# google-research/frame-interpolation

Measured on NVIDIA H100. Metric: interpolated_frames_per_sec_1080p, higher is better.
Workload: dtype f16x2-split (activations/weights as fp16 hi+lo planes; fp32 accumulate)

## Files before the change

frame_interpolation_b200/csrc/film_conv3x3_tc.cu:

```cuda
#include <cuda.h>
#include <cuda_runtime.h>
#include <stdint.h>

#include <type_traits>

#include "film_conv.h"
#include "film_tc_ptx.cuh"

namespace film {
namespace {
using namespace tc;

constexpr int kConsumers = 256;
constexpr int kThreads = kConsumers + 128;
__host__ __device__ constexpr int a_plane_bytes(int kc, int th, int tw) { return (th + 2) * tw * kc * 2; }
__host__ __device__ constexpr int a_stage_bytes(int kc, int th, int tw) { return 2 * a_plane_bytes(kc, th, tw); }
constexpr int kHaloW = 10;
__host__ __device__ constexpr int halo_box_bytes(int kc, int th) { return (th + 2) * kHaloW * kc * 2; }
__host__ __device__ constexpr int halo_plane_bytes(int kc, int th) { return (halo_box_bytes(kc, th) + 1023) & ~1023; }
__host__ __device__ constexpr int a_stage_bytes_h(int kc, int th, int tw, int halo, int planes = 2) {
  return planes * (halo ? halo_plane_bytes(kc, th) : a_plane_bytes(kc, th, tw));
}
constexpr int kMaxRing = 8;
constexpr int kSmemLimit = 227 * 1024;
constexpr int kBarBytes = 8 * (4 * kMaxRing + 4);
constexpr int kFixedBytes = kBarBytes + 16 + 512 * 4  + 64  + 1024  + 64;
constexpr int kHeadW3 = 64 * 32 * 4, kHeadMisc = 512;
constexpr int kHeadBytes = kHeadW3 + kHeadMisc;
constexpr int kPxnStageWg = 64 * 64 * 2;
constexpr int kPxnStageBytes = 2 * kPxnStageWg;
inline int epi_scratch_bytes(int epi_mode, int pxn) { return epi_mode == 3 ? kHeadBytes : pxn ? kPxnStageBytes : 0; }

__host__ __device__ inline int w_tap_bytes(int bn, int kc, int planes = 2) { return bn * kc * 2 * planes; }

template <int BN, int KC, bool kPartial, bool kHalo, bool kOne, bool kRes, bool kPxN = false>
__global__ void __launch_bounds__(kThreads, 1) k_conv3x3_tc(const ConvProblem* __restrict__ prob) {
  static_assert(!kPxN || (BN == 64 && KC == 64), "pixels on N: Cout = 64 (one M = 64 weight tile), 64-channel chunks");
  extern __shared__ uint8_t smem_raw[];
  constexpr bool one = kOne;
  const int planes = one ? 1 : 2;
  constexpr int kWPlane = BN * KC * 2;
  const int kWTap = kWPlane * planes;
  const int kTileH = prob->tile_h, kTileW = prob->tile_w;
  constexpr int kHaloTileH = kPxN ? 32 : 16;
  constexpr int kHaloBox = halo_box_bytes(KC, kHaloTileH), kHaloPlane = halo_plane_bytes(KC, kHaloTileH);
  constexpr bool halo = kHalo;
  const int kAPlane = halo ? kHaloPlane : a_plane_bytes(KC, kTileH, kTileW);
  const int kAStage = planes * kAPlane;
  const int kRowStep = kTileW * KC * 2;
  constexpr bool kFused = BN <= 128 && !kPxN;
  constexpr int kAccRegs = kPxN ? 64 : (kFused ? 2 * BN : BN) / 2;
  constexpr int kWgPx = kPxN ? 128 : 64;

  const int NA = prob->v2_na, NW = prob->v2_nw;
  const bool resident = prob->v2_resident != 0;
  const int nsrc = prob->nsrc;
  const int tiles_x = prob->tiles_x, tiles_per_img = prob->tiles_y * prob->tiles_x;
  const int cout = prob->cout;
  const int n_nt = (cout + BN - 1) / BN;
  const int ntiles = prob->B * tiles_per_img * n_nt;
  constexpr int kStageTaps = kHalo ? 9 : 3;
  constexpr bool kPacked = kPartial && kPxN;
  const int part_lo = prob->v2_part_lo, part_hi = prob->v2_part_hi;
  int nab = 0;
  for (int s = 0; s < nsrc; ++s) nab += prob->src[s].nchunk * (kHalo ? 1 : 3);
  const int nkb = nab * kStageTaps - (kPacked ? (part_hi - part_lo) * (kStageTaps - kStageTaps / 3) : 0);

  const FastDiv div_nt(n_nt, ntiles), div_img(tiles_per_img, ntiles), div_tx(tiles_x, ntiles);
  const bool pair = prob->pair != 0;
  const int rank = pair ? (int)cluster_ctarank() : 0;
  const int nsp = prob->B * tiles_per_img;
  const int nwork = pair ? ((nsp + 1) / 2) * n_nt : ntiles;
  const int w_first = pair ? (int)blockIdx.x >> 1 : (int)blockIdx.x, w_step = pair ? (int)gridDim.x >> 1 : (int)gridDim.x;
  auto decode = [&](int work, int& sp, int& nti) {
    div_nt.divmod(work, sp, nti);
    if (pair) sp = 2 * sp + rank;
  };

  const uint32_t raw = smem_u32(smem_raw);
  const uint32_t base = (raw + 1023u) & ~1023u;
  uint8_t* gen_base = smem_raw + (base - raw);
  const uint32_t a_base = base;
  const uint32_t w_base = a_base + (uint32_t)NA * kAStage;
  const uint32_t w_bytes = resident ? (uint32_t)nkb * kWTap : (uint32_t)NW * kWTap;
  const uint32_t tail = w_base + w_bytes;
  const uint32_t tail_off = (uint32_t)NA * kAStage + w_bytes;
  float* bias_smem = reinterpret_cast<float*>(gen_base + tail_off + kBarBytes + 16);
  int* src_tab = reinterpret_cast<int*>(gen_base + tail_off + kBarBytes + 16 + 512 * 4);

// ... 67 lines not shown
        __syncwarp();
      }
      int kb = 0, ab = 0;
      for (int s = 0; s < nsrc; ++s) {
        const int nchunk = src_tab[2 * s], c_off = src_tab[2 * s + 1];
        const int bs = src_tab[2 * kMaxSrc + s] ? prob->B - 1 - b : b;
        const CUtensorMap* tm_hi = &prob->tm_a_hi[s];
        const CUtensorMap* tm_lo = &prob->tm_a_lo[s];
        for (int ch = 0; ch < nchunk; ++ch) {
          const int nst = halo ? 1 : 3;
          for (int dx = 0; dx < nst; ++dx, ++ab) {
            const int st = ra.stage;
            mbar_wait(tail + 8u * (kMaxRing + st), ra.phase ^ 1u);
            if (elect_one()) {
              const uint32_t sa = a_base + st * kAStage, bar = tail + 8u * st;
              mbar_expect_tx(bar, halo ? (uint32_t)(planes * kHaloBox) : (uint32_t)kAStage);
              tma_load_4d(sa, tm_hi, bar, c_off + ch * KC, x0 + dx - 1, y0 - 1, bs);
              if (!one) tma_load_4d(sa + kAPlane, tm_lo, bar, c_off + ch * KC, x0 + dx - 1, y0 - 1, bs);
            }
            __syncwarp();
            ra.advance(NA);
            if (!resident) {
              const bool packed = kPacked && ab >= part_lo && ab < part_hi;
              const int nblk = packed ? kStageTaps / 3 : kStageTaps;
              for (int t = 0; t < nblk; ++t, ++kb) {
                const int ws = rw.stage;
                mbar_wait(tail + 8u * (3 * kMaxRing + ws), rw.phase ^ 1u);
                if (elect_one()) {
                  const uint32_t sw = w_base + ws * kWTap, bar = tail + 8u * (2 * kMaxRing + ws);
                  mbar_expect_tx(bar, kWTap);
                  if (pair) {
                    const uint32_t hoff = (uint32_t)(rank * (kWPlane / 2));
                    tma_load_2d_mc(sw + hoff, &prob->tm_w_hi_half, bar, kb * KC, n0 + rank * (BN / 2), 3);
                    if (!one) tma_load_2d_mc(sw + kWPlane + hoff, &prob->tm_w_lo_half, bar, kb * KC, n0 + rank * (BN / 2), 3);
                  } else {
                    tma_load_2d(sw, tm_w_hi, bar, kb * KC, n0);
                    if (!one) tma_load_2d(sw + kWPlane, tm_w_lo, bar, kb * KC, n0);
                  }
                }
                __syncwarp();
                rw.advance(NW);
              }
            }
          }
        }
      }
    }
    leave();
    return;
  }

  regs_inc<232>();
  const int wg = warp >> 2;
  const int q = lane & 3;
  const int H = prob->H, W = prob->W, out_H = prob->out_H, out_W = prob->out_W, out_C = prob->out_C;
  const int out_c_off = prob->out_c_off, act = prob->act;
  sp_t* const out_hi = prob->out_hi;
  sp_t* const out_lo = prob->out_lo;
  sp_t* const pool_hi = prob->pool_hi;
  sp_t* const pool_lo = prob->pool_lo;
  const int pool_C = prob->pool_C;
  const bool do_pool = pool_hi != nullptr;
  const bool lo_skip = prob->out_lo_skip != 0;
  const bool rgb = prob->epi_mode == 2;
  const float* const head_w = prob->head_w4;
  float* const rgb_out = prob->head_v;
  const int crop_y = prob->crop_y, crop_x = prob->crop_x, crop_h = prob->crop_h, crop_w = prob->crop_w;
  const int64_t crop_pitch = prob->crop_pitch;
  const bool fhead = prob->epi_mode == 3;
  constexpr int kHid = BN <= 64 ? BN / 2 : 1;
  float* const w3s = reinterpret_cast<float*>(reinterpret_cast<uint8_t*>(src_tab) + 64);
  float* const hmisc = w3s + kHeadW3 / 4;
  if (fhead) {
    if constexpr (BN <= 64) {
      for (int i = threadIdx.x; i < BN * kHid; i += kConsumers) w3s[i] = prob->head_w3[i];
      for (int i = threadIdx.x; i < kHid; i += kConsumers) hmisc[i] = prob->head_b3[i];
      for (int i = threadIdx.x; i < 2 * kHid; i += kConsumers) hmisc[kHid + i] = prob->head_w4[i];
      if (threadIdx.x < 2) hmisc[3 * kHid + threadIdx.x] = prob->head_b4[threadIdx.x];
    }
    asm volatile("bar.sync 1, %0;" ::"r"(kConsumers) : "memory");
  }
  const float* const head_vup = prob->head_vup;
  float* const head_res = prob->head_res;
  float* const head_vout = prob->head_v;

  if (resident) mbar_wait(tail + 8u * (2 * kMaxRing), 0);
  const bool is_leader = (threadIdx.x & 127) == 0;
  const uint32_t w_empty_peer = pair ? map_to_cta(tail + 8u * (3 * kMaxRing), (uint32_t)(rank ^ 1)) : 0u;
  auto release_w = [&](int slot) {
    mbar_arrive(tail + 8u * (3 * kMaxRing + slot));
    if (pair) mbar_arrive_cluster(w_empty_peer + 8u * slot);
  };
  {
    constexpr int kWTapC = kWPlane * (kOne ? 1 : 2);
    constexpr uint32_t kPx = KC * 2;
    const uint32_t a_row0 = kHalo ? (uint32_t)(wg * (kWgPx / 8) * kHaloW) * kPx : (uint32_t)(wg * kWgPx) * kPx;
    const uint32_t sbo = kHalo ? kHaloW * kPx : 8 * kPx;
    RingPos ra, rw;
    float acc[kAccRegs];
    for (int tile = w_first; tile < nwork; tile += w_step) {
      int kb = 0;
      int rel_a = -1, rel_w = -1;
      auto retire = [&](int next_a, int next_w) {
        wgmma_commit();
        wgmma_wait<1>();
        if (is_leader) {
          if (rel_a >= 0) mbar_arrive(tail + 8u * (kMaxRing + rel_a));
          if (rel_w >= 0) release_w(rel_w);
        }
        rel_a = next_a;
        rel_w = next_w;
      };
      auto stage = [&](auto ksteps_c, auto tpb_c) {
        constexpr int kSteps = decltype(ksteps_c)::value, kTpb = decltype(tpb_c)::value;
        constexpr int kBlocks = kStageTaps / kTpb;
        const int st = ra.stage;
        mbar_wait(tail + 8u * st, ra.phase);
        const uint32_t sa = a_base + st * kAStage + a_row0;
        const uint32_t lo_off = (uint32_t)(kHalo ? kHaloPlane : kAPlane);
        if constexpr (kRes) {
          const uint64_t a0 = make_desc_sbo<KC>(sa, sbo);
          const uint64_t lo_delta = (uint64_t)(lo_off >> 4);
          const uint64_t row_delta = (uint64_t)(kRowStep >> 4);
          const uint64_t w0 = make_desc_kc<KC>(w_base + kb * kWTapC);
          const uint32_t first = (kb == 0) ? 0u : 1u;
          wgmma_fence();
#pragma unroll
          for (int t = 0; t < kStageTaps; ++t) {
            const uint64_t a_hi = a0 + (kHalo ? (uint64_t)((((t % 3) * kHaloW + t / 3) * kPx) >> 4) : (uint64_t)t * row_delta);
            const uint64_t a_lo = a_hi + lo_delta;
            const uint64_t w_hi = w0 + (uint64_t)(((t / kTpb) * kWTapC + (t % kTpb) * kSteps * 32) >> 4);
            const uint64_t w_lo = w_hi + (uint64_t)(kWPlane >> 4);
#pragma unroll
            for (int k = 0; k < kSteps; ++k) {
              const uint64_t adv = (uint64_t)(k * 32 >> 4);
              const uint32_t accf = (t == 0 && k == 0) ? first : 1u;
              if constexpr (kPxN) {
                wgmma<128>(acc, w_hi + adv, a_hi + adv, accf);
                if constexpr (!kOne) {
                  wgmma<128>(acc, w_lo + adv, a_hi + adv, 1u);
                  wgmma<128>(acc, w_hi + adv, a_lo + adv, 1u);
                }
              } else if constexpr (kOne) {
                wgmma<BN>(acc, a_hi + adv, w_hi + adv, accf);
              } else if constexpr (kFused) {
                wgmma<BN>(acc, a_hi + adv, w_hi + adv, accf);
                wgmma<BN>(acc + BN / 2, a_hi + adv, w_lo + adv, accf);
                wgmma<BN>(acc, a_lo + adv, w_hi + adv, 1u);
              } else {
                wgmma<BN>(acc, a_lo + adv, w_hi + adv, accf);
                wgmma<BN>(acc, a_hi + adv, w_lo + adv, 1u);
                wgmma<BN>(acc, a_hi + adv, w_hi + adv, 1u);
              }
            }
          }
          retire(st, -1);
          kb += kBlocks;
        } else {
          for (int blk = 0; blk < kBlocks; ++blk, ++kb) {
            uint32_t sw;
            int ws = -1;
            if (resident) {
              sw = w_base + kb * kWTap;
            } else {
              ws = rw.stage;
              mbar_wait(tail + 8u * (2 * kMaxRing + ws), rw.phase);
              sw = w_base + ws * kWTap;
            }
            const uint32_t first = (kb == 0) ? 0u : 1u;
            wgmma_fence();
#pragma unroll
            for (int u = 0; u < kTpb; ++u) {
              const int t = blk * kTpb + u;
              const uint32_t off = kHalo ? (uint32_t)((t % 3) * kHaloW + t / 3) * kPx : (uint32_t)(t * kRowStep);
              const uint64_t a_hi = make_desc_sbo<KC>(sa + off, sbo);
              const uint64_t a_lo = make_desc_sbo<KC>(sa + lo_off + off, sbo);
              const uint64_t wk = (uint64_t)((u * kSteps * 32) >> 4);
// ... 22 lines not shown
              }
            }
            retire(blk == kBlocks - 1 ? st : -1, ws);
            if (!resident) rw.advance(NW);
          }
        }
        ra.advance(NA);
      };
      using Full = std::integral_constant<int, KC / 16>;
      using One = std::integral_constant<int, 1>;
      if constexpr (kPartial) {
        for (int ab = 0; ab < part_lo; ++ab) stage(Full{}, One{});
        for (int ab = part_lo; ab < part_hi; ++ab) stage(One{}, std::integral_constant<int, kPacked ? 3 : 1>{});
        for (int ab = part_hi; ab < nab; ++ab) stage(Full{}, One{});
      } else {
        for (int ab = 0; ab < nab; ++ab) stage(Full{}, One{});
      }
      wgmma_wait<0>();
      if (is_leader) {
        if (rel_a >= 0) mbar_arrive(tail + 8u * (kMaxRing + rel_a));
        if (rel_w >= 0) release_w(rel_w);
      }
      acc_fence<kAccRegs>(acc);

      int sp, nti, b, rem, ty, tx;
      decode(tile, sp, nti);
      div_img.divmod(sp, b, rem);
      div_tx.divmod(rem, ty, tx);
      const int n0 = nti * BN;
      const bool live = sp < nsp;
      if constexpr (kPxN) {
        const int c0 = 16 * (warp & 3) + (lane >> 2);
        const float bias0 = bias_smem[c0], bias1 = bias_smem[c0 + 8];
#pragma unroll
        for (int i = 0; i < kAccRegs; ++i) {
          const float f = acc[i] + ((i & 2) ? bias1 : bias0);
          acc[i] = act ? leaky(f) : f;
        }
        const int y_wg = ty * kTileH + 16 * wg, x_t = tx * kTileW;
        if (do_pool) {
          const int px = x_t + 2 * q;
#pragma unroll
          for (int j = 0; j < 16; j += 2) {
            const int py = y_wg + j;
            const bool ok = live && (py >> 1) < (out_H >> 1) && (px >> 1) < (out_W >> 1) && !(lane & 4);
            const int64_t ppix = ((int64_t)b * (out_H >> 1) + (py >> 1)) * (out_W >> 1) + (px >> 1);
#pragma unroll
            for (int h = 0; h < 2; ++h) {
              const int i = 4 * j + 2 * h;
              const float v = ((acc[i] + acc[i + 1]) + (acc[i + 4] + acc[i + 5])) * 0.25f;
              const float vn = __shfl_xor_sync(0xffffffffu, v, 4);
              if (ok) {
                uint32_t hi, lo;
// ... 295 lines not shown
    if (kPxN && (h.pair || h.tile_h != 32 || h.tile_w != 8 || h.epi_mode != 0)) return cudaErrorInvalidValue;
    const bool partial = h.v2_part_hi > h.v2_part_lo;
    const int idx = (partial ? 8 : 0) | (h.halo ? 4 : 0) | (h.passes == 1 ? 2 : 0) | (h.v2_resident && h.straight ? 1 : 0);
    if (!h.pair) {
      kFn[idx]<<<h.v2_grid, kThreads, smem_bytes_for(h, BN), st>>>(d_prob);
      return cudaGetLastError();
    }
    cudaLaunchConfig_t cfg = {};
    cudaLaunchAttribute attr[1];
    attr[0].id = cudaLaunchAttributeClusterDimension;
    attr[0].val.clusterDim.x = 2;
    attr[0].val.clusterDim.y = 1;
    attr[0].val.clusterDim.z = 1;
    cfg.gridDim = dim3(h.v2_grid);
    cfg.blockDim = dim3(kThreads);
    cfg.dynamicSmemBytes = smem_bytes_for(h, BN);
    cfg.stream = st;
    cfg.attrs = attr;
    cfg.numAttrs = 1;
    return cudaLaunchKernelEx(&cfg, kFn[idx], d_prob);
  }
};

cudaError_t conv3x3_tc_configure() {
  cudaError_t e;
#define FILM_CFG(BN, KC)                        \
  e = Variants<BN, KC>::configure();            \
  if (e != cudaSuccess) return e;
  FILM_CFG(32, 64) FILM_CFG(64, 64) FILM_CFG(128, 64) FILM_CFG(256, 64) FILM_CFG(32, 32) FILM_CFG(64, 32)
#undef FILM_CFG
  e = Variants<64, 64, true>::configure();
  if (e != cudaSuccess) return e;
  return cudaSuccess;
}

cudaError_t launch_conv3x3_tc(const ConvProblem* d_prob, const ConvProblem& h, cudaStream_t st) {
  const int bn = h.bn;
  if (h.kchunk == 32) {
    if (bn == 32) return Variants<32, 32>::launch(d_prob, h, st);
    if (bn == 64) return Variants<64, 32>::launch(d_prob, h, st);
    return cudaErrorInvalidValue;
  }
  switch (bn) {
    case 256: return Variants<256, 64>::launch(d_prob, h, st);
    case 128: return Variants<128, 64>::launch(d_prob, h, st);
    case 64: return h.pxn ? Variants<64, 64, true>::launch(d_prob, h, st) : Variants<64, 64>::launch(d_prob, h, st);
    default: return Variants<32, 64>::launch(d_prob, h, st);
  }
}

}
```

frame_interpolation_b200/csrc/film_engine.cu:

```cuda
#include <cuda.h>
#include <cuda_runtime.h>

#include <algorithm>
#include <cmath>
#include <cstdio>
#include <cstdlib>
#include <cstring>
#include <functional>
#include <map>
#include <memory>
#include <string>
#include <vector>

#include "../../include/film_b200.h"
#include "film_conv.h"
#include "film_kernels.h"
#include "film_pack.h"

namespace film {
int conv_tc_block_n(int cout);

constexpr int kLevels = 7, kFusionLevels = 5, kSpecialized = 3, kSubLevels = 4, kFilters = 64;
static const int kFlowFilters[4] = {32, 64, 128, 256};
static const char* kPredictorNames[4] = {"flow_predictor_0", "flow_predictor_1", "flow_predictor_2",
// ... 171 lines not shown
#endif
}
static float sp_to_f32(uint16_t h) {
#ifdef FILM_SPLIT_FP16
  __half v;
  memcpy(&v, &h, 2);
  return __half2float(v);
#else
  return bf16_to_f32(h);
#endif
}

struct PackedConv {
  sp_t* w_hi = nullptr;
  sp_t* w_lo = nullptr;
  float* bias = nullptr;
  int cout = 0, ktot = 0, cin_ref = 0;
  int kchunk = kChunk;
  std::vector<int> src_chunks;
  std::vector<int> src_ksteps;
  sp_t* pxn_hi = nullptr;
  sp_t* pxn_lo = nullptr;
  int pxn_ktot = 0;
  int ntaps = 0;
  int tap_dy[kMaxTaps], tap_dx[kMaxTaps];
};

struct TapSpec {
  int dy, dx;
  std::vector<std::pair<int, int>> terms;
};

static PackedConv pack_conv(const HostTensor& kernel, const HostTensor& bias,
                            const std::vector<std::vector<int>>& src_maps,
                            const std::vector<TapSpec>& taps, std::vector<void*>& allocs, int chunk = kChunk) {
  const int kw = kernel.dims[1], cin = kernel.dims[2], cout = kernel.dims[3];
  PackedConv pc;
  pc.cout = cout;
  pc.cin_ref = cin;
  pc.kchunk = chunk;
  pc.ntaps = (int)taps.size();
  for (size_t t = 0; t < taps.size(); ++t) {
    pc.tap_dy[t] = taps[t].dy;
    pc.tap_dx[t] = taps[t].dx;
  }
  int ktot = 0;
// ... 28 lines not shown
            lo[(size_t)n * ktot + kbase + c] = l;
          }
        }
      }
    }
  }
  auto upload = [&](const std::vector<uint16_t>& v) {
    sp_t* d;
    FILM_CUDA(cudaMalloc(&d, v.size() * 2));
    allocs.push_back(d);
    FILM_CUDA(cudaMemcpy(d, v.data(), v.size() * 2, cudaMemcpyHostToDevice));
    return d;
  };
  pc.w_hi = upload(hi);
  pc.w_lo = upload(lo);
  pc.pxn_hi = pc.w_hi;
  pc.pxn_lo = pc.w_lo;
  pc.pxn_ktot = ktot;
  std::vector<int> packed;
  for (int ks : pc.src_ksteps) packed.push_back(taps.size() == 9 && chunk == kChunk && ks == 1);
  if (std::count(packed.begin(), packed.end(), 1)) {
    pc.pxn_hi = upload(pack_dx_blocks(hi, cout, ktot, chunk, pc.src_chunks, packed, pc.pxn_ktot));
    pc.pxn_lo = upload(pack_dx_blocks(lo, cout, ktot, chunk, pc.src_chunks, packed, pc.pxn_ktot));
  }
  FILM_CUDA(cudaMalloc(&pc.bias, cout * 4));
  allocs.push_back(pc.bias);
  FILM_CUDA(cudaMemcpy(pc.bias, bias.data.data(), cout * 4, cudaMemcpyHostToDevice));
  return pc;
}

static std::vector<TapSpec> taps_3x3() {
  std::vector<TapSpec> t;
  for (int kx = 0; kx < 3; ++kx)
    for (int ky = 0; ky < 3; ++ky) t.push_back({ky - 1, kx - 1, {{ky, kx}}});
  return t;
}
static std::vector<TapSpec> taps_up2x2(int py, int px) {
  std::vector<TapSpec> t;
  for (int dy = 0; dy <= py; ++dy)
    for (int dx = 0; dx <= px; ++dx) {
      TapSpec s{dy, dx, {}};
      for (int fy = 0; fy < 2; ++fy)
        for (int fx = 0; fx < 2; ++fx)
          if ((py + fy) / 2 == dy && (px + fx) / 2 == dx) s.terms.push_back({fy, fx});
      t.push_back(s);
    }
// ... 175 lines not shown
};

struct Plan {
  int h, w, H, W, off_y, off_x;
  Options opt;
  int num_sms = 132;
  bool onepass(int stage) const { return stage >= 0 && opt.conv_impl == 0 && (((uint32_t)opt.onepass_mask >> stage) & 1u); }
  bool hi_only(int consumer) const { return opt.plane_skip && onepass(consumer); }
  std::vector<void*> allocs;
  int64_t arena_bytes = 0;
  std::vector<ConvProblem> h_probs;
  ConvProblem* d_probs = nullptr;
  struct Op {
    std::function<cudaError_t(cudaStream_t)> fn;
    int category;
    std::string name;
    double flops;
    double bytes;
    int lane;
    std::vector<int> waits;
    std::vector<int> signals;
    std::string form = "";
    int passes = 0;
  };
  std::vector<Op> ops;
  std::vector<float> op_ms;
  static constexpr int kNumLanes = 8;
  int cur_lane = 0, num_tokens = 0, tok_end = -1;
  std::vector<int> pending_waits;
  int new_token() { return num_tokens++; }
  void add_op(int category, const std::string& name, std::function<cudaError_t(cudaStream_t)> fn,
              double flops = 0, double bytes = 0) {
    ops.push_back(Op{std::move(fn), category, name, flops, bytes, cur_lane, pending_waits, {}});
    pending_waits.clear();
  }
  void signal_last(int token) { ops.back().signals.push_back(token); }
  std::map<std::string, DebugTensor> debug;
  float* xin = nullptr;
  float* xout = nullptr;
  float* time = nullptr;
  cudaGraphExec_t graph = nullptr;
  double conv_flops = 0, mma_flops = 0, warp_bytes = 0, last_conv_bytes = 0;
  bool times = false;
  size_t tail_begin = 0;
  int tok_head = -1;
  cudaGraphExec_t graph_tail = nullptr;
// ... 74 lines not shown
  cp.passes = P.onepass(stage) ? 1 : 3;
  cp.out_lo_skip = (!pool_out && P.hi_only(consumer)) ? 1 : 0;
  cp.straight = o.mma_straight;
  const SplitBuf* s0 = sources[0].buf;
  cp.nsrc = (int)sources.size();
  if (cp.nsrc != (int)pc.src_chunks.size()) throw Error{FILM_ERR_WEIGHTS, "source count mismatch"};
  cp.B = s0->B;
  cp.H = s0->H;
  cp.W = s0->W;
  const int kc = pc.kchunk;
  cp.kchunk = kc;
  const bool v2 = o.conv3x3_v2 && o.conv_impl == 0 && pc.ntaps == 9 && (out || epi_mode >= 2) && sy == 1 && sx == 1 &&
                  (kc == kChunk || pc.cout <= 64);
  cp.epi_mode = epi_mode;
  const auto waves = [&](long tiles) { return (tiles + P.num_sms - 1) / P.num_sms; };
  const long pxn_tiles = (long)cp.B * ((cp.H + 31) / 32) * ((cp.W + 7) / 8);
  const long tiles16 = (long)cp.B * ((cp.H + 15) / 16) * ((cp.W + 7) / 8);
  bool skips_ksteps = false;
  for (size_t s = 0; s < pc.src_chunks.size(); ++s)
    if (pc.src_chunks[s] > 0 && pc.src_ksteps[s] != kc / 16) skips_ksteps = true;
  const bool pxn_pays = skips_ksteps ? 2 * waves(pxn_tiles) <= waves(tiles16) : pxn_tiles >= 2L * P.num_sms;
  cp.pxn = (v2 && o.conv3x3_pxn && pc.cout == 64 && kc == kChunk && epi_mode == 0 && out && out_c_off % 8 == 0 &&
            out->C % 8 == 0 && (!pool_out || pool_out->C % 8 == 0) && (o.conv3x3_pxn >= 2 || pxn_pays)) ? 1 : 0;
  const int ktot = cp.pxn ? pc.pxn_ktot : pc.ktot;
  const sp_t* w_hi = cp.pxn ? pc.pxn_hi : pc.w_hi;
  const sp_t* w_lo = cp.pxn ? pc.pxn_lo : pc.w_lo;
  int box_h, box_w;
  if (v2) {
    if (cp.pxn) {
      cp.tile_h = 32;
      cp.tile_w = 8;
    } else if (pool_out) {
      cp.tile_h = 16;
      cp.tile_w = 8;
    } else {
      conv3x3_tc_pick_tile(cp.H, cp.W, cp.B, pc.cout, kc, cp.passes, ktot, epi_mode, P.num_sms, cp.tile_h, cp.tile_w);
    }
    box_h = cp.tile_h + 2;
    box_w = cp.tile_w;
  } else {
    pick_tile(cp.H, cp.W, cp.tile_h, cp.tile_w);
    box_h = cp.tile_h;
    box_w = cp.tile_w;
  }
  cp.tiles_y = (cp.H + cp.tile_h - 1) / cp.tile_h;
  cp.tiles_x = (cp.W + cp.tile_w - 1) / cp.tile_w;
  for (int s = 0; s < cp.nsrc; ++s) {
    const SplitBuf* b = sources[s].buf;
    if (b->B != cp.B || b->H != cp.H || b->W != cp.W) throw Error{FILM_ERR_ARG, "conv source grid mismatch"};
    cp.src[s].hi = b->hi;
    cp.src[s].lo = b->lo;
    cp.src[s].C = b->C;
    cp.src[s].c_off = sources[s].c_off;
    cp.src[s].nchunk = pc.src_chunks[s];
    cp.src[s].bswap = sources[s].bswap;
    if (sources[s].c_off + pc.src_chunks[s] * kc > b->C) throw Error{FILM_ERR_ARG, "conv source channel overrun"};
    make_act_map(&cp.tm_a_hi[s], b->hi, b->B, b->H, b->W, b->C, box_h, box_w, kc);
    make_act_map(&cp.tm_a_lo[s], b->lo, b->B, b->H, b->W, b->C, box_h, box_w, kc);
  }
  cp.ntaps = pc.ntaps;
  for (int t = 0; t < pc.ntaps; ++t) {
    cp.tap_dy[t] = pc.tap_dy[t];
    cp.tap_dx[t] = pc.tap_dx[t];
  }
  cp.ktot = ktot;
  cp.w_hi = w_hi;
  cp.w_lo = w_lo;
  cp.bias = pc.bias;
  cp.cout = pc.cout;
  cp.act = act;
  int bn = conv_tc_block_n(pc.cout);
  if (out && !pool_out) {
    auto items = [&](int b) { return (long)cp.B * cp.tiles_y * cp.tiles_x * ((pc.cout + b - 1) / b); };
    while (bn > 64 && 2 * items(bn) <= P.num_sms) bn /= 2;
  }
  cp.bn = bn;
  make_w_map(&cp.tm_w_hi, w_hi, pc.cout, ktot, bn, kc);
  make_w_map(&cp.tm_w_lo, w_lo, pc.cout, ktot, bn, kc);
  make_w_map(&cp.tm_w_hi_half, w_hi, pc.cout, ktot, bn / 2, kc);
  make_w_map(&cp.tm_w_lo_half, w_lo, pc.cout, ktot, bn / 2, kc);
  if (out) {
    cp.out_hi = out->hi;
    cp.out_lo = out->lo;
    cp.out_C = out->C;
    cp.out_H = out->H;
    cp.out_W = out->W;
  } else {
    cp.out_C = 0;
    cp.out_H = cp.H;
    cp.out_W = cp.W;
  }
  cp.out_c_off = out_c_off;
  cp.out_sy = sy;
  cp.out_sx = sx;
  cp.out_oy = oy;
  cp.out_ox = ox;
  if (out && (out->B != cp.B || out_c_off + pc.cout > out->C)) throw Error{FILM_ERR_ARG, "conv destination mismatch"};
  if (pool_out) {
    if (!v2) throw Error{FILM_ERR_UNSUPPORTED, "fused pool needs the persistent 3x3 kernel"};
    cp.pool_hi = pool_out->hi;
    cp.pool_lo = pool_out->lo;
    cp.pool_C = pool_out->C;
  }
  cp.group = 1;
  int halo_ok = (v2 && cp.tile_h == (cp.pxn ? 32 : 16) && cp.tile_w == 8) ? o.conv3x3_halo : 0;
  if (kc != kChunk && halo_ok < 3) halo_ok = 0;
  if (cp.pxn && skips_ksteps) halo_ok = 0;
  cp.halo = halo_ok >= 2;
  if (v2 && !conv3x3_tc_plan(cp, P.num_sms))
    throw Error{FILM_ERR_UNSUPPORTED, "persistent 3x3 conv: shared-memory rings do not fit (" + tag + ")"};
  if (v2 && o.conv3x3_2cta && epi_mode < 2 && !cp.v2_resident && !cp.pxn &&
      (o.conv3x3_2cta >= 2 || (long)cp.B * cp.tiles_y * cp.tiles_x >= 4L * P.num_sms)) {
    cp.pair = 1;
    if (halo_ok >= 1) cp.halo = 1;
    if (!conv3x3_tc_plan(cp, P.num_sms))
      throw Error{FILM_ERR_UNSUPPORTED, "persistent 3x3 conv: shared-memory rings do not fit (" + tag + ")"};
  }
  if (cp.halo) {
    for (int s = 0; s < cp.nsrc; ++s) {
      const SplitBuf* b = sources[s].buf;
      make_act_map(&cp.tm_a_hi[s], b->hi, b->B, b->H, b->W, b->C, box_h, box_w + 2, kc);
      make_act_map(&cp.tm_a_lo[s], b->lo, b->B, b->H, b->W, b->C, box_h, box_w + 2, kc);
    }
  }
  if (v2) {
    const int nst = cp.halo ? 1 : 3;
    for (int s = 0, ab = 0; s < cp.nsrc; ab += pc.src_chunks[s] * nst, ++s) {
      if (pc.src_chunks[s] == 0 || pc.src_ksteps[s] == kc / 16) continue;
      if (pc.src_ksteps[s] != 1 || cp.v2_part_hi > cp.v2_part_lo)
        throw Error{FILM_ERR_UNSUPPORTED, "persistent 3x3 conv: only one source may skip k-steps, and it must issue one (" +
                                              tag + ")"};
      cp.v2_part_lo = ab;
      cp.v2_part_hi = ab + pc.src_chunks[s] * nst;
    }
  }
  const size_t idx = P.h_probs.size();
  P.h_probs.push_back(cp);
  double k_issued = 0;
  for (size_t si = 0; si < pc.src_chunks.size(); ++si)
    k_issued += (double)pc.src_chunks[si] * pc.ntaps * (v2 ? pc.src_ksteps[si] * 16 : pc.kchunk);
  P.mma_flops += (double)cp.passes * 2.0 * (double)cp.B * cp.tiles_y * cp.tiles_x * (cp.tile_h * cp.tile_w) * k_issued *
                 (double)(((pc.cout + bn - 1) / bn) * bn);
  double alg_bytes = 0;
  {
    const double px = (double)cp.B * cp.H * cp.W, planes_in = cp.passes == 1 ? 1.0 : 2.0;
    for (size_t si = 0; si < pc.src_chunks.size(); ++si) alg_bytes += px * pc.src_chunks[si] * pc.kchunk * 2.0 * planes_in;
    if (out) alg_bytes += px * pc.cout * 2.0 * (cp.out_lo_skip ? 1.0 : 2.0);
    if (pool_out) alg_bytes += px / 4.0 * pc.cout * 4.0;
    if (epi_mode == 2) alg_bytes += px * 12.0;
    if (!out && epi_mode != 2) alg_bytes += px * 24.0;
    alg_bytes += (double)pc.cout * ktot * 2.0 * planes_in;
  }
  P.last_conv_bytes = alg_bytes;
  if (out && sy == 1 && sx == 1 && !tag.empty())
    P.debug["out:" + tag] = DebugTensor{true, out->hi, out->lo, out->pixels(), out->C, out_c_off, pc.cout};
  if (pool_out)
    P.debug["pool:" + tag] = DebugTensor{true, pool_out->hi, pool_out->lo, pool_out->pixels(), pool_out->C, 0, pc.cout};
  if (no_op) return idx;
  Plan* pp = &P;
  const int impl = o.conv_impl;
  P.add_op(0, tag, [pp, idx, impl, v2](cudaStream_t st) {
    if (impl == 1) return launch_conv_simt(pp->d_probs + idx, pp->h_probs[idx], st);
    return v2 ? launch_conv3x3_tc(pp->d_probs + idx, pp->h_probs[idx], st)
              : launch_conv_tc(pp->d_probs + idx, pp->h_probs[idx], st);
  }, 2.0 * ref_macs_per_px * (double)cp.B * cp.H * cp.W, alg_bytes);
  P.ops.back().form = impl == 1 ? "simt" : !v2 ? "tc" : cp.pxn ? "3x3_pxn" : cp.pair ? "3x3_pair" : "3x3";
  P.ops.back().passes = cp.passes;
  return idx;
}

static void padded_size(int h, int w, int align, int& H, int& W, int& off_y, int& off_x) {
  int ph = 0, pw = 0;
  if (align > 0) {
    ph = (h % align) ? align - h % align : 0;
    pw = (w % align) ? align - w % align : 0;
  }
  H = h + ph;
  W = w + pw;
  off_y = ph / 2;
  off_x = pw / 2;
}

static std::unique_ptr<Plan> build_plan(const Model& M, int h, int w, int align, const Options& opt, int num_sms,
                                        bool times) {
  std::unique_ptr<Plan> pl(new Plan);
  Plan& P = *pl;
  P.opt = opt;
  P.times = times;
  P.reuse = !opt.keep_debug && !opt.use_lanes && opt.arena_reuse;
  const bool fuse_rgb = opt.conv_impl == 0 && opt.conv3x3_v2 && opt.fuse_rgb_head;
// ... 162 lines not shown
                        C, 0, C};
        P.debug["flow_vup" + std::to_string(d) + "/" + std::to_string(l)] =
            DebugTensor{false, vup + (int64_t)d * hh * ww * 2, nullptr, (int64_t)hh * ww, 2, 0, 2};
      }
    }
    const int cpad = round_up(nf, nf < kChunk ? 32 : kChunk);
    SplitBuf* c0 = P.split(2, hh, ww, cpad);
    SplitBuf* c1 = P.split(2, hh, ww, cpad);
    SplitBuf* c2 = P.split(2, hh, ww, cpad);
    const std::string lt = "@L" + std::to_string(l);
    std::vector<SrcRef> flow_src(2);
    flow_src[0].buf = feat[l];
    flow_src[0].c_off = 0;
    flow_src[1].buf = second ? second : feat[l];
    flow_src[1].c_off = 0;
    flow_src[1].bswap = second ? 0 : 1;
    add_conv(P, "flow_conv0" + lt, 9.0 * 2 * C * nf, M.flow[p][0], flow_src, 1, c0, 0, ST_FLOW_L0 + l, ST_FLOW_L0 + l);
    add_conv(P, "flow_conv1" + lt, 9.0 * nf * nf, M.flow[p][1], {{c0, 0}}, 1, c1, 0, ST_FLOW_L0 + l, ST_FLOW_L0 + l);
    const bool fuse_head = opt.conv_impl == 0 && opt.conv3x3_v2 && opt.fuse_flow_head && nf <= (opt.fuse_flow_head >= 2 ? 64 : 32);
    if (fuse_head) {
      const size_t ci = add_conv(P, "flow_conv2+head" + lt, 9.0 * nf * nf + 1.0 * nf * (nf / 2) + (nf / 2) * 2.0, M.flow[p][2],
                                 {{c1, 0}}, 1, nullptr, 0, ST_FLOW_L0 + l, ST_NONE, 1, 1, 0, 0, nullptr, false, 3);
      ConvProblem& hp = P.h_probs[ci];
      if (hp.bn != nf) throw Error{FILM_ERR_UNSUPPORTED, "flow-head epilogue expects one N tile on the single-CTA kernel"};
      hp.head_w3 = M.flow_w3[p];
      hp.head_b3 = M.flow_b3[p];
      hp.head_w4 = M.flow_w4[p];
      hp.head_b4 = M.flow_b4[p];
      hp.head_vup = vup;
      hp.head_res = res[l];
      hp.head_v = v[l];
    } else {
      add_conv(P, "flow_conv2" + lt, 9.0 * nf * nf, M.flow[p][2], {{c1, 0}}, 1, c2, 0, ST_FLOW_L0 + l, ST_NONE);
    }
    if (fuse_head) {
    } else if (opt.conv_impl == 1) {
      const float *w3 = M.flow_w3[p], *b3 = M.flow_b3[p], *w4 = M.flow_w4[p], *b4 = M.flow_b4[p];
      float *rr = res[l], *vv = v[l];
      const float* vu = vup;
      const int npix = 2 * hh * ww;
      P.add_op(2, "flow_head" + lt, [=](cudaStream_t st) {
        return launch_flow_head(c2->hi, c2->lo, c2->C, nf, npix, w3, b3, w4, b4, vu, rr, vv, st);
      });
    } else {
      const size_t ci = add_conv(P, "flow_head" + lt, 1.0 * nf * (nf / 2) + (nf / 2) * 2.0, M.flow_c3[p], {{c2, 0}}, 1,
                                 nullptr, 0, ST_NONE, ST_NONE);
      ConvProblem& hp = P.h_probs[ci];
// ... 1051 lines not shown
  return p;
}

void film_host_free(void* p) {
  if (p) cudaFreeHost(p);
}

int film_profile(film_handle* h, film_profile_t* out) {
  if (!h || !out) return FILM_ERR_ARG;
  if (h->prof.last_call_ms < 0 && h->last_plan && h->dev_events_valid) {
    float t = 0;
    if (cudaEventSynchronize(h->ev[2]) == cudaSuccess && cudaEventElapsedTime(&t, h->ev[1], h->ev[2]) == cudaSuccess)
      h->prof.last_call_ms = t;
    else
      (void)cudaGetLastError();
  }
  *out = h->prof;
  return FILM_OK;
}

int film_op_table(film_handle* h, char* buf, int64_t buf_size, int64_t* needed) {
  if (!h || !h->last_plan) return FILM_ERR_ARG;
  try {
  std::string out = "idx,category,name,ms,ref_flops,alg_bytes,form,passes\n";
  Plan* P = h->last_plan;
  for (size_t i = 0; i < P->ops.size(); ++i) {
    char line[256];
    const std::string passes = P->ops[i].passes ? std::to_string(P->ops[i].passes) : "";
    snprintf(line, sizeof(line), "%zu,%d,%s,%.6f,%.0f,%.0f,%s,%s\n", i, P->ops[i].category, P->ops[i].name.c_str(),
             i < P->op_ms.size() ? P->op_ms[i] : -1.f, P->ops[i].flops, P->ops[i].bytes, P->ops[i].form.c_str(),
             passes.c_str());
    out += line;
  }
  if (needed) *needed = (int64_t)out.size() + 1;
  if (buf && buf_size > 0) {
    const size_t n = out.size() < (size_t)buf_size - 1 ? out.size() : (size_t)buf_size - 1;
    memcpy(buf, out.data(), n);
    buf[n] = 0;
  }
  return FILM_OK;
  }
  FILM_CATCH_ALL(h)
}

int film_debug_read(film_handle* h, const char* name, float* dst, int64_t* count) {
  if (!h || !name) return FILM_ERR_ARG;
  try {
    if (!h->last_plan) throw Error{FILM_ERR_ARG, "no call has been made yet"};
    std::string base(name);
    int plane = -1;
    const size_t n_base = base.size();
    if (n_base > 3 && (base.compare(n_base - 3, 3, ".hi") == 0 || base.compare(n_base - 3, 3, ".lo") == 0)) {
      plane = base[n_base - 2] == 'h' ? 0 : 1;
      base.resize(n_base - 3);
// ... 36 lines not shown
```

frame_interpolation_b200/csrc/film_pack.h:

```cpp
#pragma once
#include <stdint.h>

#include <vector>

namespace film {

inline std::vector<uint16_t> pack_dx_blocks(const std::vector<uint16_t>& per_tap, int cout, int ktot, int chunk,
                                            const std::vector<int>& src_chunks, const std::vector<int>& packed,
                                            int& ktot_out) {
  ktot_out = ktot;
  for (size_t s = 0; s < src_chunks.size(); ++s)
    if (packed[s]) ktot_out -= src_chunks[s] * 6 * chunk;
  std::vector<uint16_t> out((size_t)cout * ktot_out, 0);
  for (int n = 0; n < cout; ++n) {
    const uint16_t* src = per_tap.data() + (size_t)n * ktot;
    uint16_t* dst = out.data() + (size_t)n * ktot_out;
    for (size_t s = 0; s < src_chunks.size(); ++s)
      for (int ch = 0; ch < src_chunks[s]; ++ch, src += 9 * chunk) {
        if (!packed[s]) {
          for (int k = 0; k < 9 * chunk; ++k) *dst++ = src[k];
          continue;
        }
        for (int t = 0; t < 9; ++t)
          for (int c = 0; c < 16; ++c) dst[(t / 3) * chunk + (t % 3) * 16 + c] = src[t * chunk + c];
        dst += 3 * chunk;
      }
  }
  return out;
}

}
```

frame_interpolation_b200/interpolator.py:

```python
from __future__ import annotations

import ctypes as C
from typing import List, Optional

import numpy as np

from . import _lib, weights as _weights


def _fptr(a: np.ndarray):
    return a.ctypes.data_as(C.POINTER(C.c_float))


def image_to_patches(image: np.ndarray, block_shape: List[int]) -> np.ndarray:
    block_height, block_width = block_shape
    height, width, channel = image.shape[-3:]
    patch_height, patch_width = height // block_height, width // block_width
    assert height == (patch_height * block_height), \
        'block_height=%d should evenly divide height=%d.' % (block_height, height)
    assert width == (patch_width * block_width), \
        'block_width=%d should evenly divide width=%d.' % (block_width, width)
    x = np.reshape(image, (block_height, patch_height, block_width, patch_width, channel))
    x = np.transpose(x, (0, 2, 1, 3, 4))
    return np.ascontiguousarray(np.reshape(x, (block_height * block_width, patch_height, patch_width, channel)))
# ... 249 lines not shown
        p = _lib.FilmProfile()
        self._check(self._lib.film_profile(self._handle, C.byref(p)))
        return {k: getattr(p, k) for k, _ in p._fields_ if k != "reserved"}

    def debug_read(self, name: str) -> np.ndarray:
        n = C.c_int64()
        self._check(self._lib.film_debug_read(self._handle, name.encode(), None, C.byref(n)))
        out = np.empty(n.value, np.float32)
        self._check(self._lib.film_debug_read(self._handle, name.encode(), _fptr(out), C.byref(n)))
        return out

    def op_table(self) -> List[dict]:
        n = C.c_int64()
        self._check(self._lib.film_op_table(self._handle, None, 0, C.byref(n)))
        buf = C.create_string_buffer(n.value)
        self._check(self._lib.film_op_table(self._handle, buf, n.value, C.byref(n)))
        rows = buf.value.decode().strip().split("\n")
        keys = rows[0].split(",")
        out = []
        for r in rows[1:]:
            v = r.split(",")
            out.append({"idx": int(v[0]), "category": int(v[1]), "name": v[2], "ms": float(v[3]),
                        "ref_flops": float(v[4]), "alg_bytes": float(v[5]), "form": v[6],
                        "passes": int(v[7]) if v[7] else None})
        return out

    @property
    def version(self) -> str:
        return self._lib.film_version().decode()
```

Before: 26.18.

## Add dy-folded pixels-on-N 3x3 conv path for 32-channel outputs

Result: faster. 26.44, median of 6 (+1.0%).

```diff
diff --git a/frame_interpolation_b200/csrc/film_conv3x3_tc.cu b/frame_interpolation_b200/csrc/film_conv3x3_tc.cu
--- a/frame_interpolation_b200/csrc/film_conv3x3_tc.cu
+++ b/frame_interpolation_b200/csrc/film_conv3x3_tc.cu
@@ -29,13 +29,19 @@
 constexpr int kHeadBytes = kHeadW3 + kHeadMisc;
 constexpr int kPxnStageWg = 64 * 64 * 2;
 constexpr int kPxnStageBytes = 2 * kPxnStageWg;
-inline int epi_scratch_bytes(int epi_mode, int pxn) { return epi_mode == 3 ? kHeadBytes : pxn ? kPxnStageBytes : 0; }
+constexpr int kFoldStageWg = 128 * 32 * 4;
+constexpr int kFoldStageBytes = 2 * kFoldStageWg;
+inline int epi_scratch_bytes(int epi_mode, int pxn) {
+  return (epi_mode == 3 ? kHeadBytes : 0) + (pxn == 2 ? kFoldStageBytes : pxn ? kPxnStageBytes : 0);
+}
 
 __host__ __device__ inline int w_tap_bytes(int bn, int kc, int planes = 2) { return bn * kc * 2 * planes; }
 
-template <int BN, int KC, bool kPartial, bool kHalo, bool kOne, bool kRes, bool kPxN = false>
+template <int BN, int KC, bool kPartial, bool kHalo, bool kOne, bool kRes, bool kPxN = false, bool kFold = false>
 __global__ void __launch_bounds__(kThreads, 1) k_conv3x3_tc(const ConvProblem* __restrict__ prob) {
-  static_assert(!kPxN || (BN == 64 && KC == 64), "pixels on N: Cout = 64 (one M = 64 weight tile), 64-channel chunks");
+  static_assert(!kPxN || (BN == 64 && (KC == 64 || kFold)), "pixels on N: one M = 64 weight tile, 64-channel chunks");
+  static_assert(!kFold || (kPxN && kHalo && kOne && kRes && !kPartial),
+                "dy-folded pixels on N: single-pass, wide halo, resident weights, no partial source");
   extern __shared__ uint8_t smem_raw[];
   constexpr bool one = kOne;
   const int planes = one ? 1 : 2;
@@ -64,7 +70,8 @@
   const int part_lo = prob->v2_part_lo, part_hi = prob->v2_part_hi;
   int nab = 0;
   for (int s = 0; s < nsrc; ++s) nab += prob->src[s].nchunk * (kHalo ? 1 : 3);
-  const int nkb = nab * kStageTaps - (kPacked ? (part_hi - part_lo) * (kStageTaps - kStageTaps / 3) : 0);
+  constexpr int kStageBlocks = kFold ? 6 : kStageTaps;
+  const int nkb = nab * kStageBlocks - (kPacked ? (part_hi - part_lo) * (kStageTaps - kStageTaps / 3) : 0);
 
   const FastDiv div_nt(n_nt, ntiles), div_img(tiles_per_img, ntiles), div_tx(tiles_x, ntiles);
   const bool pair = prob->pair != 0;
@@ -178,7 +185,7 @@
             ra.advance(NA);
             if (!resident) {
               const bool packed = kPacked && ab >= part_lo && ab < part_hi;
-              const int nblk = packed ? kStageTaps / 3 : kStageTaps;
+              const int nblk = packed ? kStageTaps / 3 : kStageBlocks;
               for (int t = 0; t < nblk; ++t, ++kb) {
                 const int ws = rw.stage;
                 mbar_wait(tail + 8u * (3 * kMaxRing + ws), rw.phase ^ 1u);
@@ -224,11 +231,19 @@
   const int crop_y = prob->crop_y, crop_x = prob->crop_x, crop_h = prob->crop_h, crop_w = prob->crop_w;
   const int64_t crop_pitch = prob->crop_pitch;
   const bool fhead = prob->epi_mode == 3;
-  constexpr int kHid = BN <= 64 ? BN / 2 : 1;
+  constexpr int kHid = kFold ? 16 : BN <= 64 ? BN / 2 : 1;
   float* const w3s = reinterpret_cast<float*>(reinterpret_cast<uint8_t*>(src_tab) + 64);
   float* const hmisc = w3s + kHeadW3 / 4;
   if (fhead) {
-    if constexpr (BN <= 64) {
+    if constexpr (kFold) {
+      for (int i = threadIdx.x; i < 32 * kHid; i += kConsumers) {
+        const int c = i / kHid, hh = i % kHid;
+        w3s[c * kHid + ((((hh >> 2) ^ (c >> 3)) & 3) << 2) + (hh & 3)] = prob->head_w3[i];
+      }
+      for (int i = threadIdx.x; i < kHid; i += kConsumers) hmisc[i] = prob->head_b3[i];
+      for (int i = threadIdx.x; i < 2 * kHid; i += kConsumers) hmisc[kHid + i] = prob->head_w4[i];
+      if (threadIdx.x < 2) hmisc[3 * kHid + threadIdx.x] = prob->head_b4[threadIdx.x];
+    } else if constexpr (BN <= 64) {
       for (int i = threadIdx.x; i < BN * kHid; i += kConsumers) w3s[i] = prob->head_w3[i];
       for (int i = threadIdx.x; i < kHid; i += kConsumers) hmisc[i] = prob->head_b3[i];
       for (int i = threadIdx.x; i < 2 * kHid; i += kConsumers) hmisc[kHid + i] = prob->head_w4[i];
@@ -254,6 +269,7 @@
     const uint32_t sbo = kHalo ? kHaloW * kPx : 8 * kPx;
     RingPos ra, rw;
     float acc[kAccRegs];
+    float acc2[kFold ? kAccRegs : 1];
     for (int tile = w_first; tile < nwork; tile += w_step) {
       int kb = 0;
       int rel_a = -1, rel_w = -1;
@@ -269,7 +285,7 @@
       };
       auto stage = [&](auto ksteps_c, auto tpb_c) {
         constexpr int kSteps = decltype(ksteps_c)::value, kTpb = decltype(tpb_c)::value;
-        constexpr int kBlocks = kStageTaps / kTpb;
+        constexpr int kBlocks = kFold ? kStageBlocks : kStageTaps / kTpb;
         const int st = ra.stage;
         mbar_wait(tail + 8u * st, ra.phase);
         const uint32_t sa = a_base + st * kAStage + a_row0;
@@ -281,6 +297,19 @@
           const uint64_t w0 = make_desc_kc<KC>(w_base + kb * kWTapC);
           const uint32_t first = (kb == 0) ? 0u : 1u;
           wgmma_fence();
+          if constexpr (kFold) {
+#pragma unroll
+            for (int t = 0; t < kStageBlocks; ++t) {
+              const uint64_t a_hi = a0 + (uint64_t)((((t & 1) * 2 * kHaloW + (t >> 1)) * kPx) >> 4);
+              const uint64_t w_hi = w0 + (uint64_t)((t * kWTapC) >> 4);
+#pragma unroll
+              for (int k = 0; k < KC / 16; ++k) {
+                const uint64_t adv = (uint64_t)(k * 32 >> 4);
+                const uint32_t accf = (t < 2 && k == 0) ? first : 1u;
+                wgmma<128>((t & 1) ? acc2 : acc, w_hi + adv, a_hi + adv, accf);
+              }
+            }
+          } else {
 #pragma unroll
           for (int t = 0; t < kStageTaps; ++t) {
             const uint64_t a_hi = a0 + (kHalo ? (uint64_t)((((t % 3) * kHaloW + t / 3) * kPx) >> 4) : (uint64_t)t * row_delta);
@@ -309,6 +338,7 @@
                 wgmma<BN>(acc, a_hi + adv, w_hi + adv, 1u);
               }
             }
+          }
           }
           retire(st, -1);
           kb += kBlocks;
@@ -377,6 +407,7 @@
         if (rel_w >= 0) release_w(rel_w);
       }
       acc_fence<kAccRegs>(acc);
+      if constexpr (kFold) acc_fence<kAccRegs>(acc2);
 
       int sp, nti, b, rem, ty, tx;
       decode(tile, sp, nti);
@@ -384,6 +415,98 @@
       div_tx.divmod(rem, ty, tx);
       const int n0 = nti * BN;
       const bool live = sp < nsp;
+      if constexpr (kFold) {
+        float* const stg = reinterpret_cast<float*>(reinterpret_cast<uint8_t*>(src_tab) + 64 + (fhead ? kHeadBytes : 0) +
+                                                    wg * kFoldStageWg);
+        const int c = 16 * (warp & 1) + (lane >> 2);
+        auto at = [](int p, int ch) { return p * 32 + (ch ^ (((p >> 1) & 3) << 3)); };
+        auto wg_sync = [&]() { asm volatile("bar.sync %0, 128;" ::"r"(2 + wg) : "memory"); };
+        wg_sync();
+        if (!(warp & 2)) {
+#pragma unroll
+          for (int i = 0; i < kAccRegs; ++i) stg[at(8 * (i >> 2) + 2 * q + (i & 1), c + 8 * ((i >> 1) & 1))] = acc[i] + acc2[i];
+        }
+        wg_sync();
+        if (warp & 2) {
+#pragma unroll
+          for (int i = 4; i < kAccRegs; ++i) stg[at(8 * (i >> 2) - 8 + 2 * q + (i & 1), c + 8 * ((i >> 1) & 1))] += acc[i];
+#pragma unroll
+          for (int i = 4 * 14; i < 4 * 15; ++i) stg[at(8 * 15 + 2 * q + (i & 1), c + 8 * ((i >> 1) & 1))] += acc2[i];
+        }
+        wg_sync();
+        const int y_wg = ty * kTileH + 16 * wg, x_t = tx * kTileW;
+        const int t128 = threadIdx.x & 127;
+#pragma unroll
+        for (int k = 0; k < 4; ++k) {
+          const int idx = 128 * k + t128, p = idx >> 2, g = idx & 3;
+          const int py = y_wg + (p >> 3), px = x_t + (p & 7);
+          const bool valid = live && py < H && px < W;
+          const int64_t opix = ((int64_t)b * out_H + py) * out_W + px;
+          const float4* s = reinterpret_cast<const float4*>(stg + at(p, 8 * g));
+          const float4 v0 = s[0], v1 = s[1];
+          float f[8] = {v0.x, v0.y, v0.z, v0.w, v1.x, v1.y, v1.z, v1.w};
+#pragma unroll
+          for (int e = 0; e < 8; ++e) {
+            f[e] += bias_smem[8 * g + e];
+            if (act) f[e] = leaky(f[e]);
+          }
+          if (fhead) {
+            float hp[kHid];
+#pragma unroll
+            for (int hh = 0; hh < kHid; ++hh) hp[hh] = 0.f;
+#pragma unroll
+            for (int e = 0; e < 8; ++e) {
+              const float4* wr = reinterpret_cast<const float4*>(w3s + (8 * g + e) * kHid);
+#pragma unroll
+              for (int h4 = 0; h4 < kHid / 4; ++h4) {
+                const float4 wv = wr[h4 ^ g];
+                hp[4 * h4] = fmaf(f[e], wv.x, hp[4 * h4]);
+                hp[4 * h4 + 1] = fmaf(f[e], wv.y, hp[4 * h4 + 1]);
+                hp[4 * h4 + 2] = fmaf(f[e], wv.z, hp[4 * h4 + 2]);
+                hp[4 * h4 + 3] = fmaf(f[e], wv.w, hp[4 * h4 + 3]);
+              }
+            }
+#pragma unroll
+            for (int hh = 0; hh < kHid; ++hh) {
+              hp[hh] += __shfl_xor_sync(0xffffffffu, hp[hh], 1);
+              hp[hh] += __shfl_xor_sync(0xffffffffu, hp[hh], 2);
+            }
+            if (g == 0 && valid) {
+              float f0 = hmisc[3 * kHid], f1 = hmisc[3 * kHid + 1];
+#pragma unroll
+              for (int hh = 0; hh < kHid; ++hh) {
+                const float x = leaky(hp[hh] + hmisc[hh]);
+                f0 = fmaf(x, hmisc[kHid + 2 * hh], f0);
+                f1 = fmaf(x, hmisc[kHid + 2 * hh + 1], f1);
+              }
+              float2 res = make_float2(f0, f1), tot = res;
+              if (head_vup) {
+                const float2 u = reinterpret_cast<const float2*>(head_vup)[opix];
+                tot.x += u.x;
+                tot.y += u.y;
+              }
+              reinterpret_cast<float2*>(head_res)[opix] = res;
+              reinterpret_cast<float2*>(head_vout)[opix] = tot;
+            }
+            continue;
+          }
+          if (!valid) continue;
+          sp_t* const oh = out_hi + opix * out_C + out_c_off + 8 * g;
+          if (lo_skip) {
+            *reinterpret_cast<uint4*>(oh) = make_uint4(pack2_hi(f[0], f[1]), pack2_hi(f[2], f[3]), pack2_hi(f[4], f[5]),
+                                                       pack2_hi(f[6], f[7]));
+          } else {
+            uint4 hv, lv;
+            split_pack2(f[0], f[1], hv.x, lv.x);
+            split_pack2(f[2], f[3], hv.y, lv.y);
+            split_pack2(f[4], f[5], hv.z, lv.z);
+            split_pack2(f[6], f[7], hv.w, lv.w);
+            *reinterpret_cast<uint4*>(oh) = hv;
+            *reinterpret_cast<uint4*>(out_lo + opix * out_C + out_c_off + 8 * g) = lv;
+          }
+        }
+        continue;
+      }
       if constexpr (kPxN) {
         const int c0 = 16 * (warp & 3) + (lane >> 2);
         const float bias0 = bias_smem[c0], bias1 = bias_smem[c0 + 8];
@@ -725,6 +848,21 @@
   }
 };
 
+template <int KC>
+struct FoldVariant {
+  static constexpr void (*kFn)(const ConvProblem*) = k_conv3x3_tc<64, KC, false, true, true, true, true, true>;
+  static cudaError_t configure() {
+    return cudaFuncSetAttribute(kFn, cudaFuncAttributeMaxDynamicSharedMemorySize, kSmemLimit);
+  }
+  static cudaError_t launch(const ConvProblem* d_prob, const ConvProblem& h, cudaStream_t st) {
+    if (h.bn != 64 || h.cout != 32 || !h.v2_resident || h.v2_na < 2 || !h.halo || h.passes != 1 || h.pair ||
+        h.tile_h != 32 || h.tile_w != 8 || (h.epi_mode != 0 && h.epi_mode != 3) || h.v2_part_hi > h.v2_part_lo)
+      return cudaErrorInvalidValue;
+    kFn<<<h.v2_grid, kThreads, smem_bytes_for(h, 64), st>>>(d_prob);
+    return cudaGetLastError();
+  }
+};
+
 cudaError_t conv3x3_tc_configure() {
   cudaError_t e;
 #define FILM_CFG(BN, KC)                        \
@@ -734,11 +872,16 @@
 #undef FILM_CFG
   e = Variants<64, 64, true>::configure();
   if (e != cudaSuccess) return e;
+  e = FoldVariant<64>::configure();
+  if (e != cudaSuccess) return e;
+  e = FoldVariant<32>::configure();
+  if (e != cudaSuccess) return e;
   return cudaSuccess;
 }
 
 cudaError_t launch_conv3x3_tc(const ConvProblem* d_prob, const ConvProblem& h, cudaStream_t st) {
   const int bn = h.bn;
+  if (h.pxn == 2) return h.kchunk == 32 ? FoldVariant<32>::launch(d_prob, h, st) : FoldVariant<64>::launch(d_prob, h, st);
   if (h.kchunk == 32) {
     if (bn == 32) return Variants<32, 32>::launch(d_prob, h, st);
     if (bn == 64) return Variants<64, 32>::launch(d_prob, h, st);
diff --git a/frame_interpolation_b200/csrc/film_engine.cu b/frame_interpolation_b200/csrc/film_engine.cu
--- a/frame_interpolation_b200/csrc/film_engine.cu
+++ b/frame_interpolation_b200/csrc/film_engine.cu
@@ -217,6 +217,9 @@
   sp_t* pxn_hi = nullptr;
   sp_t* pxn_lo = nullptr;
   int pxn_ktot = 0;
+  sp_t* fold_hi = nullptr;
+  sp_t* fold_lo = nullptr;
+  int fold_ktot = 0;
   int ntaps = 0;
   int tap_dy[kMaxTaps], tap_dx[kMaxTaps];
 };
@@ -291,6 +294,10 @@
   if (std::count(packed.begin(), packed.end(), 1)) {
     pc.pxn_hi = upload(pack_dx_blocks(hi, cout, ktot, chunk, pc.src_chunks, packed, pc.pxn_ktot));
     pc.pxn_lo = upload(pack_dx_blocks(lo, cout, ktot, chunk, pc.src_chunks, packed, pc.pxn_ktot));
+  }
+  if (cout == 32 && taps.size() == 9) {
+    pc.fold_hi = upload(pack_dy_folded(hi, ktot, chunk, pc.fold_ktot));
+    pc.fold_lo = upload(pack_dy_folded(lo, ktot, chunk, pc.fold_ktot));
   }
   FILM_CUDA(cudaMalloc(&pc.bias, cout * 4));
   allocs.push_back(pc.bias);
@@ -512,6 +519,7 @@
     std::vector<int> signals;
     std::string form = "";
     int passes = 0;
+    double mma_flops = 0;
   };
   std::vector<Op> ops;
   std::vector<float> op_ms;
@@ -632,9 +640,14 @@
   const bool pxn_pays = skips_ksteps ? 2 * waves(pxn_tiles) <= waves(tiles16) : pxn_tiles >= 2L * P.num_sms;
   cp.pxn = (v2 && o.conv3x3_pxn && pc.cout == 64 && kc == kChunk && epi_mode == 0 && out && out_c_off % 8 == 0 &&
             out->C % 8 == 0 && (!pool_out || pool_out->C % 8 == 0) && (o.conv3x3_pxn >= 2 || pxn_pays)) ? 1 : 0;
-  const int ktot = cp.pxn ? pc.pxn_ktot : pc.ktot;
-  const sp_t* w_hi = cp.pxn ? pc.pxn_hi : pc.w_hi;
-  const sp_t* w_lo = cp.pxn ? pc.pxn_lo : pc.w_lo;
+  const bool fold_store = epi_mode == 0 && out && !pool_out && out_c_off % 8 == 0 && out->C % 8 == 0;
+  if (v2 && o.conv3x3_pxn && pc.cout == 32 && pc.fold_hi && cp.passes == 1 && (fold_store || epi_mode == 3) &&
+      !skips_ksteps && o.conv3x3_halo >= (kc == kChunk ? 2 : 3) && (o.conv3x3_pxn >= 2 || pxn_tiles >= 2L * P.num_sms))
+    cp.pxn = 2;
+  const int ktot = cp.pxn == 2 ? pc.fold_ktot : cp.pxn ? pc.pxn_ktot : pc.ktot;
+  const sp_t* w_hi = cp.pxn == 2 ? pc.fold_hi : cp.pxn ? pc.pxn_hi : pc.w_hi;
+  const sp_t* w_lo = cp.pxn == 2 ? pc.fold_lo : cp.pxn ? pc.pxn_lo : pc.w_lo;
+  const int w_rows = cp.pxn == 2 ? 64 : pc.cout;
   int box_h, box_w;
   if (v2) {
     if (cp.pxn) {
@@ -679,16 +692,16 @@
   cp.bias = pc.bias;
   cp.cout = pc.cout;
   cp.act = act;
-  int bn = conv_tc_block_n(pc.cout);
+  int bn = cp.pxn == 2 ? 64 : conv_tc_block_n(pc.cout);
   if (out && !pool_out) {
     auto items = [&](int b) { return (long)cp.B * cp.tiles_y * cp.tiles_x * ((pc.cout + b - 1) / b); };
     while (bn > 64 && 2 * items(bn) <= P.num_sms) bn /= 2;
   }
   cp.bn = bn;
-  make_w_map(&cp.tm_w_hi, w_hi, pc.cout, ktot, bn, kc);
-  make_w_map(&cp.tm_w_lo, w_lo, pc.cout, ktot, bn, kc);
-  make_w_map(&cp.tm_w_hi_half, w_hi, pc.cout, ktot, bn / 2, kc);
-  make_w_map(&cp.tm_w_lo_half, w_lo, pc.cout, ktot, bn / 2, kc);
+  make_w_map(&cp.tm_w_hi, w_hi, w_rows, ktot, bn, kc);
+  make_w_map(&cp.tm_w_lo, w_lo, w_rows, ktot, bn, kc);
+  make_w_map(&cp.tm_w_hi_half, w_hi, w_rows, ktot, bn / 2, kc);
+  make_w_map(&cp.tm_w_lo_half, w_lo, w_rows, ktot, bn / 2, kc);
   if (out) {
     cp.out_hi = out->hi;
     cp.out_lo = out->lo;
@@ -719,6 +732,8 @@
   cp.halo = halo_ok >= 2;
   if (v2 && !conv3x3_tc_plan(cp, P.num_sms))
     throw Error{FILM_ERR_UNSUPPORTED, "persistent 3x3 conv: shared-memory rings do not fit (" + tag + ")"};
+  if (cp.pxn == 2 && (!cp.halo || !cp.v2_resident))
+    throw Error{FILM_ERR_UNSUPPORTED, "dy-folded pixels on N needs the wide halo and resident weights (" + tag + ")"};
   if (v2 && o.conv3x3_2cta && epi_mode < 2 && !cp.v2_resident && !cp.pxn &&
       (o.conv3x3_2cta >= 2 || (long)cp.B * cp.tiles_y * cp.tiles_x >= 4L * P.num_sms)) {
     cp.pair = 1;
@@ -749,8 +764,9 @@
   double k_issued = 0;
   for (size_t si = 0; si < pc.src_chunks.size(); ++si)
     k_issued += (double)pc.src_chunks[si] * pc.ntaps * (v2 ? pc.src_ksteps[si] * 16 : pc.kchunk);
-  P.mma_flops += (double)cp.passes * 2.0 * (double)cp.B * cp.tiles_y * cp.tiles_x * (cp.tile_h * cp.tile_w) * k_issued *
-                 (double)(((pc.cout + bn - 1) / bn) * bn);
+  const double op_mma_flops = (double)cp.passes * 2.0 * (double)cp.B * cp.tiles_y * cp.tiles_x * (cp.tile_h * cp.tile_w) *
+                              k_issued * (double)(((pc.cout + bn - 1) / bn) * bn) * (cp.pxn == 2 ? 6.0 / 9.0 : 1.0);
+  P.mma_flops += op_mma_flops;
   double alg_bytes = 0;
   {
     const double px = (double)cp.B * cp.H * cp.W, planes_in = cp.passes == 1 ? 1.0 : 2.0;
@@ -776,6 +792,7 @@
   }, 2.0 * ref_macs_per_px * (double)cp.B * cp.H * cp.W, alg_bytes);
   P.ops.back().form = impl == 1 ? "simt" : !v2 ? "tc" : cp.pxn ? "3x3_pxn" : cp.pair ? "3x3_pair" : "3x3";
   P.ops.back().passes = cp.passes;
+  P.ops.back().mma_flops = op_mma_flops;
   return idx;
 }
 
@@ -984,7 +1001,8 @@
       const size_t ci = add_conv(P, "flow_conv2+head" + lt, 9.0 * nf * nf + 1.0 * nf * (nf / 2) + (nf / 2) * 2.0, M.flow[p][2],
                                  {{c1, 0}}, 1, nullptr, 0, ST_FLOW_L0 + l, ST_NONE, 1, 1, 0, 0, nullptr, false, 3);
       ConvProblem& hp = P.h_probs[ci];
-      if (hp.bn != nf) throw Error{FILM_ERR_UNSUPPORTED, "flow-head epilogue expects one N tile on the single-CTA kernel"};
+      if (hp.bn != (hp.pxn == 2 ? 64 : nf))
+        throw Error{FILM_ERR_UNSUPPORTED, "flow-head epilogue expects one N tile on the single-CTA kernel"};
       hp.head_w3 = M.flow_w3[p];
       hp.head_b3 = M.flow_b3[p];
       hp.head_w4 = M.flow_w4[p];
@@ -2082,14 +2100,14 @@
 int film_op_table(film_handle* h, char* buf, int64_t buf_size, int64_t* needed) {
   if (!h || !h->last_plan) return FILM_ERR_ARG;
   try {
-  std::string out = "idx,category,name,ms,ref_flops,alg_bytes,form,passes\n";
+  std::string out = "idx,category,name,ms,ref_flops,alg_bytes,form,passes,mma_flops\n";
   Plan* P = h->last_plan;
   for (size_t i = 0; i < P->ops.size(); ++i) {
     char line[256];
     const std::string passes = P->ops[i].passes ? std::to_string(P->ops[i].passes) : "";
-    snprintf(line, sizeof(line), "%zu,%d,%s,%.6f,%.0f,%.0f,%s,%s\n", i, P->ops[i].category, P->ops[i].name.c_str(),
+    snprintf(line, sizeof(line), "%zu,%d,%s,%.6f,%.0f,%.0f,%s,%s,%.0f\n", i, P->ops[i].category, P->ops[i].name.c_str(),
              i < P->op_ms.size() ? P->op_ms[i] : -1.f, P->ops[i].flops, P->ops[i].bytes, P->ops[i].form.c_str(),
-             passes.c_str());
+             passes.c_str(), P->ops[i].mma_flops);
     out += line;
   }
   if (needed) *needed = (int64_t)out.size() + 1;
diff --git a/frame_interpolation_b200/csrc/film_pack.h b/frame_interpolation_b200/csrc/film_pack.h
--- a/frame_interpolation_b200/csrc/film_pack.h
+++ b/frame_interpolation_b200/csrc/film_pack.h
@@ -29,4 +29,23 @@
   return out;
 }
 
+inline std::vector<uint16_t> pack_dy_folded(const std::vector<uint16_t>& per_tap, int ktot, int chunk, int& ktot_out) {
+  constexpr int kCout = 32;
+  const int nchunk = ktot / (9 * chunk);
+  ktot_out = nchunk * 6 * chunk;
+  std::vector<uint16_t> out((size_t)2 * kCout * ktot_out);
+  for (int r = 0; r < 2 * kCout; ++r) {
+    const int n = r % kCout;
+    for (int cb = 0; cb < nchunk; ++cb)
+      for (int blk = 0; blk < 6; ++blk) {
+        const int dx = blk / 2;
+        const int ky = r >= kCout ? 1 : (blk % 2) * 2;
+        const uint16_t* src = per_tap.data() + (size_t)n * ktot + ((size_t)cb * 9 + 3 * dx + ky) * chunk;
+        uint16_t* dst = out.data() + (size_t)r * ktot_out + ((size_t)cb * 6 + blk) * chunk;
+        for (int c = 0; c < chunk; ++c) dst[c] = src[c];
+      }
+  }
+  return out;
 }
+
+}
diff --git a/frame_interpolation_b200/interpolator.py b/frame_interpolation_b200/interpolator.py
--- a/frame_interpolation_b200/interpolator.py
+++ b/frame_interpolation_b200/interpolator.py
@@ -295,7 +295,7 @@
             v = r.split(",")
             out.append({"idx": int(v[0]), "category": int(v[1]), "name": v[2], "ms": float(v[3]),
                         "ref_flops": float(v[4]), "alg_bytes": float(v[5]), "form": v[6],
-                        "passes": int(v[7]) if v[7] else None})
+                        "passes": int(v[7]) if v[7] else None, "mma_flops": float(v[8])})
         return out
 
     @property
```
